# Rongjiehuang/FastDiff

Measured on AMD Instinct MI355X. Metric: real-time factor (audio-sec/wall-sec), N=4 reverse steps, 80x864 mel, higher is better.
Workload: dtype f32 results; 2-piece fp16 operands (22 bit) on fp16 MFMA, fp32 accumulate; GEMM as Winograd F(2,3); exact-fp32 twin; 1 GPU; BASELINE configs[1]: LJSpeech shape, batch=8 x 80x864 mel per GPU, N=4, HIP kernels + hipGraph sampler; batch_per_gpu=8, frames=864, reverse_steps=4, graph=True, weights=random init seed 1234 (no checkpoint offline), world_size=1, gpus_visible=1, oversubscribed=False

## Files before the change

fastdiff_amd/_capi.py:

```python
import ctypes as ct
import os

_HERE = os.path.dirname(os.path.abspath(__file__))
LIB_PATH = os.path.join(_HERE, "lib", "libfastdiff_hip.so")

FD_OK, FD_ERR_INVALID, FD_ERR_UNSUPPORTED, FD_ERR_HIP, FD_ERR_STATE, FD_ERR_MISSING = 0, -1, -2, -3, -4, -5


class FdConfig(ct.Structure):
    _fields_ = [("audio_channels", ct.c_int), ("inner_channels", ct.c_int), ("cond_channels", ct.c_int),
                ("n_upsample", ct.c_int), ("upsample_ratios", ct.c_int * 8), ("lvc_layers_each_block", ct.c_int),
                ("lvc_kernel_size", ct.c_int), ("kpnet_hidden_channels", ct.c_int), ("kpnet_conv_size", ct.c_int),
                ("diffusion_step_embed_dim_in", ct.c_int), ("diffusion_step_embed_dim_mid", ct.c_int),
                ("diffusion_step_embed_dim_out", ct.c_int), ("use_weight_norm", ct.c_int)]


class FdStep(ct.Structure):
    _fields_ = [("t", ct.c_float), ("c_eps", ct.c_float), ("c_div", ct.c_float), ("sigma", ct.c_float),
                ("c1", ct.c_float), ("c2", ct.c_float), ("c3", ct.c_float), ("add_noise", ct.c_int32)]


class FdWeightRef(ct.Structure):
    _fields_ = [("name", ct.c_char_p), ("data", ct.c_void_p), ("dims", ct.POINTER(ct.c_int64)), ("ndim", ct.c_int32), ("reserved", ct.c_int32)]


class FdKernelStat(ct.Structure):
    _fields_ = [("name", ct.c_char * 48), ("launches", ct.c_int64), ("total_ms", ct.c_double)]


class FdEmaItem(ct.Structure):
    _fields_ = [("p", ct.c_void_p), ("e", ct.c_void_p), ("numel", ct.c_int64)]


class FdEmaHyper(ct.Structure):
    _fields_ = [("decay", ct.c_double), ("warmup", ct.c_double)]


class FdEmaState(ct.Structure):
    _fields_ = [("updates", ct.c_uint64), ("seen_applied", ct.c_uint64), ("w", ct.c_float), ("apply", ct.c_int32)]


def step_table(rows):
    steps = (FdStep * len(rows))()
    for k, row in enumerate(rows):
        steps[k] = FdStep(float(row["t"]), float(row["c_eps"]), float(row["c_div"]), float(row["sigma"]),
                          float(row["c1"]), float(row["c2"]), float(row["c3"]), int(row["add_noise"]))
    return steps


EXPORTS = ["fd_default_config", "fd_create", "fd_destroy", "fd_last_error", "fd_set_weight", "fd_commit_weights",
           "fd_forward", "fd_sample", "fd_sample_check", "fd_sample_ticket", "fd_sample_settle", "fd_set_noise_streams", "fd_sample_halo_frames", "fd_sample_span", "fd_peak_normalize_int16", "fd_peak_normalize_int16_ragged", "fd_mel_spectrogram", "fd_set_mel_filterbank", "fd_get_mel_filterbank", "fd_lvc_forward", "fd_lvc_backward", "fd_lvc_forward_strided", "fd_lvc_backward_strided", "fd_gate_forward", "fd_gate_backward", "fd_kconv_forward", "fd_kconv_backward", "fd_weight_norm_multi_forward", "fd_weight_norm_multi_backward", "fd_refresh_weights_device", "fd_get_weight_image", "fd_get_weight_flags", "fd_pack_source", "fd_fan_forward", "fd_fan_backward", "fd_input_conv_forward", "fd_input_conv_backward", "fd_kconv_backward_w_multi", "fd_kconv_forward_act_multi", "fd_kconv_backward_x_multi", "fd_input_conv_forward_multi", "fd_input_conv_backward_multi", "fd_kconv_forward_act", "fd_kconv_backward_act", "fd_kconv_forward_frames", "fd_kconv_backward_frames", "fd_lvc_forward_frames", "fd_lvc_backward_frames", "fd_conv32_forward", "fd_conv32_backward", "fd_weight_norm_forward", "fd_weight_norm_backward", "fd_conv7_forward", "fd_conv7_backward", "fd_upsample_forward", "fd_upsample_backward", "fd_train_draw", "fd_train_collate", "fd_eval_collate", "fd_item_distance", "fd_eval_accumulate", "fd_mse_forward", "fd_mse_backward", "fd_adamw_multi", "fd_ema_multi", "fd_set_option", "fd_read_tap", "fd_kernel_index", "fd_bias_index",
           "fd_get_profile", "fd_reset_profile", "fd_get_counter", "fd_version", "fd_abi_revision"]

_lib = None


class FastDiffHipError(RuntimeError):
    pass


def load():
    global _lib
    if _lib is not None:
        return _lib
    if not os.path.exists(LIB_PATH):
        raise FastDiffHipError(
            f"{LIB_PATH} is missing: build it with `python -m fastdiff_amd.build` (hipcc, gfx950). "
            "fastdiff_amd has no CPU fallback.")
    lib = ct.CDLL(LIB_PATH)
    vp, ci, cf = ct.c_void_p, ct.c_int, ct.c_float
    lib.fd_version.restype = ct.c_char_p
    lib.fd_last_error.restype = ct.c_char_p
    lib.fd_last_error.argtypes = [vp]
    lib.fd_default_config.argtypes = [ct.POINTER(FdConfig)]
    lib.fd_create.argtypes = [ct.POINTER(FdConfig), ci, ct.POINTER(vp)]
    lib.fd_destroy.argtypes = [vp]
    lib.fd_set_weight.argtypes = [vp, ct.c_char_p, vp, ct.POINTER(ct.c_int64), ci]
    lib.fd_commit_weights.argtypes = [vp]
    lib.fd_refresh_weights_device.argtypes = [vp, ct.POINTER(FdWeightRef), ci, vp]
    lib.fd_get_weight_image.argtypes = [vp, vp, ct.POINTER(ct.c_size_t)]
    lib.fd_get_weight_flags.argtypes = [vp, ct.POINTER(ct.c_uint)]
    lib.fd_pack_source.argtypes = [ct.c_char_p, ci, ci, ci]
    lib.fd_forward.argtypes = [vp, vp, vp, vp, ci, ci, vp, vp, vp]
    lib.fd_sample.argtypes = [vp, vp, ci, ci, vp, ct.POINTER(FdStep), ci, ci, vp, vp, ct.c_uint64, vp, vp, vp]
# ... 27 lines not shown
    lib.fd_kconv_forward_act_multi.argtypes = [vp, ci, vp, vp, vp, ci, ci, ci, ct.c_float, vp, vp]
    lib.fd_kconv_backward_x_multi.argtypes = [vp, ci, vp, vp, vp, vp, ci, ci, ci, ct.c_float, ct.c_float, vp, vp]
    lib.fd_input_conv_forward_multi.argtypes = [vp, ci, vp, vp, vp, ci, ci, ct.c_float, vp, vp]
    lib.fd_input_conv_backward_multi.argtypes = [vp, ci, vp, vp, vp, vp, ci, ci, ct.c_float, vp, vp, vp, vp]
    lib.fd_kconv_backward_w_multi.argtypes = [vp, ci, vp, vp, vp, ci, ci, ci, ct.c_float, vp, vp, vp]
    lib.fd_kconv_forward_frames.argtypes = [vp, vp, vp, vp, ci, ci, ci, vp, vp]
    lib.fd_kconv_backward_frames.argtypes = [vp, vp, vp, vp, ci, ci, ci, vp, vp, vp, vp]
    lib.fd_lvc_forward_frames.argtypes = [vp, vp, vp, ct.c_int64, vp, ct.c_int64, ci, ci, ci, vp, vp]
    lib.fd_lvc_backward_frames.argtypes = [vp, vp, vp, ct.c_int64, vp, ci, ci, ci, vp, vp, ct.c_int64, vp, ct.c_int64, vp]
    lib.fd_conv32_forward.argtypes = [vp, vp, vp, vp, vp, ci, ct.c_int64, ci, cf, cf, vp, vp, vp]
    lib.fd_conv32_backward.argtypes = [vp, vp, vp, vp, vp, vp, ci, ct.c_int64, ci, cf, cf, vp, vp, vp, vp]
    lib.fd_conv7_forward.argtypes = [vp, ci, vp, vp, vp, ci, ct.c_int64, vp, vp]
    lib.fd_conv7_backward.argtypes = [vp, ci, vp, vp, vp, ci, ct.c_int64, vp, vp, vp, vp]
    lib.fd_upsample_forward.argtypes = [vp, vp, vp, vp, ci, ct.c_int64, ci, vp, vp]
    lib.fd_upsample_backward.argtypes = [vp, vp, vp, vp, ci, ct.c_int64, ci, vp, vp, vp, vp]
    lib.fd_weight_norm_forward.argtypes = [vp, vp, vp, ct.c_int64, ci, vp, vp, vp]
    lib.fd_weight_norm_backward.argtypes = [vp, vp, vp, vp, vp, ct.c_int64, ci, vp, vp, vp]
    lib.fd_gate_forward.argtypes = [vp, vp, vp, ci, ci, ct.c_int64, vp, vp]
    lib.fd_gate_backward.argtypes = [vp, vp, vp, ci, ci, ct.c_int64, vp, vp]
    lib.fd_train_draw.argtypes = [vp, vp, vp, ci, ci, ct.c_int64, ct.c_uint64, vp, ct.c_uint64, vp, vp, vp, vp]
    lib.fd_train_collate.argtypes = [vp, vp, vp, vp, ct.c_int64, ci, ci, ci, ct.c_uint64, vp, ct.c_uint64, ci, ci, vp, vp, vp, vp]
    lib.fd_eval_collate.argtypes = [vp, vp, vp, vp, ct.c_int64, ci, ci, ci, ct.c_uint64, vp, ct.c_uint64, vp, vp, vp, vp]
    lib.fd_item_distance.argtypes = [vp, vp, vp, ci, ct.c_int64, ci, vp, vp]
    lib.fd_eval_accumulate.argtypes = [vp, vp, vp, vp, ci, ci, ci, vp, vp, vp, vp]
    lib.fd_mse_forward.argtypes = [vp, vp, vp, ct.c_int64, vp, vp, vp]
    lib.fd_mse_backward.argtypes = [vp, vp, vp, vp, ct.c_int64, vp, vp]
    lib.fd_adamw_multi.argtypes = [vp, vp, ci, vp, vp, vp]
    lib.fd_ema_multi.argtypes = [vp, vp, ci, vp, vp, vp, vp]
    lib.fd_set_option.argtypes = [vp, ct.c_char_p, ct.c_char_p]
    lib.fd_read_tap.argtypes = [vp, ct.c_char_p, vp, ct.c_int64]
    lib.fd_read_tap.restype = ct.c_int64
    lib.fd_kernel_index.argtypes = [ci, ci, ci, ci]
    lib.fd_bias_index.argtypes = [ci, ci]
    lib.fd_get_profile.argtypes = [vp, ct.POINTER(FdKernelStat), ci]
    lib.fd_reset_profile.argtypes = [vp]
    lib.fd_get_counter.argtypes = [vp, ct.c_char_p]
    lib.fd_get_counter.restype = ct.c_int64
    _lib = lib
    return lib


def check(lib, handle, rc, what):
    if rc >= 0:
        return rc
    msg = lib.fd_last_error(handle)
    msg = msg.decode() if msg else what
    if rc == FD_ERR_INVALID:
        raise AssertionError(msg)
    if rc == FD_ERR_UNSUPPORTED:
        raise NotImplementedError(msg)
    if rc == FD_ERR_MISSING:
        raise KeyError(msg)
    raise FastDiffHipError(f"{what}: {msg} (status {rc})")
```

fastdiff_amd/csrc/fd_api_ext.cpp:

```cpp
#include <math.h>
#include <stddef.h>
#include <stdlib.h>
#include <string.h>

#include <algorithm>

#include "fd_kernels.h"
#include "fd_host.h"

extern "C" {

static const int MEL_NM = 80, MEL_NB = 513;
static std::vector<float> default_mel_bank(int variant)
{
    const double sr = 22050.0;
    const double f_sp = 200.0 / 3, min_log_hz = 1000.0, min_log_mel = min_log_hz / f_sp, logstep = log(6.4) / 27.0;
    auto hz_to_mel = [&](double f) { return f >= min_log_hz ? min_log_mel + log(f / min_log_hz) / logstep : f / f_sp; };
    auto mel_to_hz = [&](double m) { return m >= min_log_mel ? min_log_hz * exp(logstep * (m - min_log_mel)) : f_sp * m; };
    const double band[MEL_VARIANTS][2] = {{80.0, 7600.0}, {0.0, 8000.0}};
    std::vector<double> mf(MEL_NM + 2);
    const double m0 = hz_to_mel(band[variant][0]), m1 = hz_to_mel(band[variant][1]);
    for (int i = 0; i < MEL_NM + 2; ++i) mf[i] = mel_to_hz(m0 + (m1 - m0) * i / (MEL_NM + 1));
    std::vector<float> fb((size_t)MEL_NM * MEL_NB, 0.0f);
    for (int m = 0; m < MEL_NM; ++m) {
// ... 175 lines not shown
        n = (int64_t)B * T * fd::KREC; src = w.kpack + (k[5] - '0') * n;
    } else if (k.size() == 5 && k.compare(0, 4, "kp_h") == 0 && k[4] >= '0' && k[4] <= '2') {
        n = (int64_t)B * fd::HID * T; src = w.kp_hB + (k[4] - '0') * n;
    } else if (k.size() == 2 && k[0] == 'x' && k[1] >= '0' && k[1] <= '2') {
        if (!h->mode.keep_taps) FD_FAIL(h, FD_ERR_STATE, "fd_read_tap: set option taps=1 before the forward to keep block outputs");
        const int blk = k[1] - '0';
        src = w.xtap[blk]; n = (int64_t)B * fd::C * T * fd::hop(blk);
    } else if (k == "range_flags") {
        src = reinterpret_cast<const float *>(w.range_flag); n = 32;
    } else if (k == "range_flags_call") {
        src = reinterpret_cast<const float *>(w.range_flag + 64); n = 32;
    } else FD_FAIL(h, FD_ERR_INVALID, "fd_read_tap: unknown tap '%s'", name);
    if (!host_dst) return n;
    if (capacity < n) FD_FAIL(h, FD_ERR_INVALID, "fd_read_tap: capacity %lld < %lld", (long long)capacity, (long long)n);
    FD_HIP(h, hipSetDevice(h->device));
    FD_HIP(h, hipDeviceSynchronize());
    FD_HIP(h, hipMemcpy(host_dst, src, sizeof(float) * n, hipMemcpyDeviceToHost));
    return n;
}

int fd_kernel_index(int layer, int in_ch, int out_ch, int tap)
{
    if (layer < 0 || layer >= fd::LAYERS || in_ch < 0 || in_ch >= fd::C || out_ch < 0 || out_ch >= 2 * fd::C || tap < 0 || tap >= 3)
        return FD_ERR_INVALID;
    return fd::kernel_index(layer, in_ch, out_ch, tap);
}

int fd_bias_index(int layer, int out_ch)
{
    if (layer < 0 || layer >= fd::LAYERS || out_ch < 0 || out_ch >= 2 * fd::C) return FD_ERR_INVALID;
    return fd::bias_index(layer, out_ch);
}

int64_t fd_get_counter(fd_handle h, const char *name)
{
    if (!h || !name) return FD_ERR_INVALID;
    const std::string k(name);
    if (k == "pieces_redone" || k == "fp32_mask") {
        const int rcs = fd_settle(h);
        if (rcs != FD_OK) return rcs;
    }
    if (k == "pieces") return h->n_pieces;
    if (k == "pieces_redone") return h->n_pieces_redone;
    if (k == "pieces_fp32") return h->n_pieces_fp32;
    if (k == "fp32_mask") return (int64_t)h->call_fp32_mask;
    if (k == "calls_redone") return h->n_calls_redone;
    if (k == "graph_captures") return h->n_graph_captures;
    if (k == "graph_hits") return h->n_graph_hits;
    if (k == "graph_evictions") return h->n_graph_evictions;
    if (k == "weight_refreshes") return h->n_refreshes;
    if (k == "refresh_graph_drops") return h->n_refresh_graph_drops;
    if (k == "graphs_resident") return (int64_t)h->graphs.size();
    if (k == "graphs_retired") return (int64_t)h->retired.size();
    if (k == "workspace_bytes") return (int64_t)(h->ws.bytes + h->span_scratch.bytes);
    FD_FAIL(h, FD_ERR_INVALID, "fd_get_counter: unknown counter '%s'", name);
}

int fd_get_profile(fd_handle h, fd_kernel_stat *stats, int capacity)
{
    if (!h) return FD_ERR_INVALID;
    hipSetDevice(h->device);
    fd_prof_drain(h);
    int i = 0;
    for (const auto &kv : h->prof_acc) {
        if (stats && i < capacity) {
            memset(&stats[i], 0, sizeof(fd_kernel_stat));
            strncpy(stats[i].name, kv.first.c_str(), sizeof(stats[i].name) - 1);
            stats[i].launches = kv.second.first;
            stats[i].total_ms = kv.second.second;
        }
        ++i;
    }
    return i;
}

int fd_reset_profile(fd_handle h)
{
    if (!h) return FD_ERR_INVALID;
    fd_prof_drain(h);
    h->prof_acc.clear();
    return FD_OK;
}

}
```

fastdiff_amd/csrc/fd_internal.h:

```cpp
#pragma once
#include <hip/hip_runtime.h>
#include <hip/hip_ext.h>
#include <stdint.h>
#include <string.h>
#include <map>
#include <string>
#include <vector>

#include "../../include/fastdiff_hip.h"
#include "../../include/fastdiff_hip_ext.h"
#include "../../include/fastdiff_hip_train.h"

namespace fd {
constexpr int C = 32;
constexpr int COND = 80;
constexpr int HID = 64;
constexpr int NBLK = 3;
constexpr int LAYERS = 4;
constexpr int HOPT = 256;
constexpr int E_IN = 128, E_MID = 512, E_OUT = 512;
constexpr int KLAYER = 2 * C * C * 3;
constexpr int KW = KLAYER * LAYERS;
constexpr int KB = 2 * C * LAYERS;
constexpr int KREC = KW + KB;
// ... 208 lines not shown
    bool defer_check = false;
    static constexpr int STAGE_SLOTS = 8;
    struct StageSlot { char *host = nullptr; size_t cap = 0; hipEvent_t done = nullptr; };
    StageSlot stage[STAGE_SLOTS];
    unsigned stage_next = 0;
    struct SampleArgs {
        const float *mel = nullptr;
        int B = 0, T = 0, N = 0, ddim = 0;
        bool has_lens = false;
        std::vector<int> lens;
        std::vector<fd_step> table;
        const float *x_T = nullptr, *z = nullptr;
        unsigned long long seed = 0;
        float *out = nullptr, *seq_out = nullptr;
        hipStream_t stream = nullptr;
        std::vector<unsigned long long> ids;
        std::vector<long long> offs;
    };
    struct PendingCall {
        bool active = false;
        bool lazy = false;
        int slot = 0;
        long long ticket = 0;
        int B = 0, T = 0, N = 0, first = 0, count = 0;
        int T_io = 0;
        float *out = nullptr;
        hipStream_t stream = nullptr;
        StepMode mode;
        SampleArgs args;
    } pending;
    long long ticket_counter = 0;
    long long n_pieces = 0, n_pieces_redone = 0, n_pieces_fp32 = 0, n_calls_redone = 0;
    unsigned call_fp32_mask = 0;
    long long redone_ring[16] = {};
    unsigned redone_next = 0;
    int *flags_host = nullptr;
    hipEvent_t flags_done = nullptr, flags_done2 = nullptr;
    void *scratch = nullptr;
    Scratch lvc_scratch;
    Scratch kconv_scratch;
    Scratch cconv_scratch;
    Scratch span_scratch;
    Scratch step_scratch;
    std::vector<ProfEntry> prof_pending;
    std::vector<hipEvent_t> event_pool;
    std::map<std::string, std::pair<int64_t, double>> prof_acc;
};

enum Pipe { PIPE_F16_THEN_F32, PIPE_F16_ONLY, PIPE_F32_ONLY };
inline Pipe fd_pipe(const StepMode &m, bool f16_possible, int flag_word)
{
    if (!f16_possible || ((m.fp32_mask >> flag_word) & 1u)) return PIPE_F32_ONLY;
    return m.inline_fallback ? PIPE_F16_THEN_F32 : PIPE_F16_ONLY;
}
inline bool front_writes_h_image(const StepMode &m, const DevWeights &w)
{
    return m.fast[ST_KP_FRONT] && fd_pipe(m, m.conv_f16 && w.kpf_f16_ok, 19) != PIPE_F32_ONLY &&
           fd_pipe(m, m.gemm_f16 && w.gemm_f16_ok, 0) != PIPE_F32_ONLY && !(m.gemm_wino && w.gemm_w_ok);
}
inline bool last_lvc_fuses_final(const StepMode &m, const DevWeights &w)
{
    return m.fast[ST_LVC] && m.fast[ST_FINAL] && !m.keep_taps && m.fuse_final &&
           fd_pipe(m, m.lvc_f16 && w.lvc_f16_ok, 1 + 2 * fd::LAYERS + 3) != PIPE_F32_ONLY;
}

struct StepIO {
// ... 60 lines not shown
```

fastdiff_amd/csrc/fd_kernels.h:

```cpp
#pragma once
#include "fd_internal.h"

namespace fdk_fast {
constexpr int GX_CT = 4;
constexpr int GX_ROWB = 2 * 128;
constexpr int GW_PAIRS = 32;
constexpr int GW_ROWB = 1024;
__host__ __device__ inline int gx_rows(int T) { return ((T + GX_CT * 32 - 1) / (GX_CT * 32)) * (GX_CT * 32) + 2; }
__host__ __device__ inline int gw_pairs(int T) { return ((T + 2 * GW_PAIRS - 1) / (2 * GW_PAIRS)) * GW_PAIRS; }
}

namespace fdk {
hipError_t naive_first_conv(const Launch &L, const StepIO &io, int B, int T);
hipError_t naive_dblock(const Launch &L, int d, int B, int T);
hipError_t naive_kp_front(const Launch &L, const StepIO &io, int B, int T);
hipError_t naive_kp_gemm(const Launch &L, int B, int T);
hipError_t naive_convt(const Launch &L, int n, const float *x_in, float *x_out, int B, int Lin);
hipError_t naive_lvc_layer(const Launch &L, int n, int layer, float *x, const float *skip, float *y, int B, int T);
hipError_t naive_final_eps(const Launch &L, const float *x32, float *eps, int B, int T);
hipError_t naive_update(const Launch &L, float *x, const float *eps, int64_t n);
hipError_t fast_first_conv(const Launch &L, const StepIO &io, int B, int T);
hipError_t fast_dblock(const Launch &L, int d, int B, int T, const float *audio);
hipError_t fast_kp_front(const Launch &L, const StepIO &io, int B, int T);
hipError_t fast_kp_gemm(const Launch &L, int B, int T);
hipError_t fast_convt(const Launch &L, int n, const float *x_in, float *x_out, int B, int Lin);
hipError_t fast_lvc_layer(const Launch &L, const StepIO &io, int n, int layer, const float *x_in, const float *skip, float *x_out, int B, int T,
                          bool up = false);
hipError_t fast_final(const Launch &L, const StepIO &io, const float *x32, int B, int T);
bool lvc_op_needs_scratch(int Cin, int Cout, int ks, int hop);
hipError_t lvc_op_forward(const Launch &L, const float *x, const float *K, const float *bias, float *out, int B, int Cin, int Cout, int ks,
                          int T, int hop, float *scratch, int64_t kbs = 0, bool frames = false, int64_t bbs = 0);
hipError_t lvc_op_backward(const Launch &L, const float *x, const float *K, const float *dout, float *dx, float *dK, float *dbias, int B,
                           int Cin, int Cout, int ks, int T, int hop, float *scratch, int64_t kbs = 0, int64_t dkbs = 0, bool frames = false,
                           int64_t dbbs = 0);
hipError_t gate_forward(const Launch &L, const float *x, const float *y, float *out, int B, int C, int64_t len);
hipError_t gate_backward(const Launch &L, const float *y, const float *dout, float *dy, int B, int C, int64_t len);
hipError_t fan_pick(const Launch &L, const float *x, float *out, int rows, int64_t len, int f);
hipError_t fan_sum(const Launch &L, const float *const g[4], const float *gp, float *dx, int rows, int64_t len, int f);
bool kconv_supported(int M, int T);
size_t kconv_scratch_floats(int B, int M, int T);
bool kconv_frames_supported(int M, int T);
bool kconv_act_supported(int M, int T);
// ... 89 lines not shown
```

fastdiff_amd/csrc/fd_kernels_kp.hip:

```cpp
#include "fd_kernels_common.h"

namespace fdk_fast {

constexpr int KPF_VALID = 48, KPF_LDI = 68, KPF_LDH = 66;

struct KpFrontW {
    const float *in_pack[fd::NBLK], *in_b[fd::NBLK];
    const float *res_pack[fd::NBLK][6], *res_b[fd::NBLK][6];
};

__global__ void __launch_bounds__(256, 2) k_kp_front(const float *__restrict__ mel, float *__restrict__ hout, KpFrontW w,
                                                     const float *__restrict__ noise, const StepParams *params, int sampler,
                                                     int B, int T, const int *__restrict__ run_if, const int *__restrict__ lens)
{
    __shared__ float xin[fd::COND * KPF_LDI];
    if (run_if && *run_if == 0) return;
    __shared__ float h0[fd::HID * KPF_LDH];
    __shared__ float hA[fd::HID * KPF_LDH];
    __shared__ float hB[fd::HID * KPF_LDH];
    const int blk = blockIdx.z, b = blockIdx.y, t0 = blockIdx.x * KPF_VALID;
    const int Tb = frames_of(lens, b, T);
    if (t0 >= Tb) return;
    const int tid = threadIdx.x, lane = tid & 63, wave = tid >> 6, l31 = lane & 31, hi = lane >> 5;
    const int mt = wave & 1, nt = wave >> 1;
// ... 597 lines not shown
                const float bv = gb[ptile * 32 + l31] * GX_SCALE;
#pragma unroll
                for (int r = 0; r < 16; ++r) bias_lo[r] = bv;
                have_blk = cur.blk; have_xg = cur.xg;
                __builtin_amdgcn_s_waitcnt(0x0F70);
            }
            const bool more = (i + half + 1 < n_mine);
            GX_WALK_NEXT(walk, cur, more, nxt, run, left);
            const int Tb = frames_of(lens, cur.b, T);
            const bool full = (Tb % 32 == 0) || (cur.chunk * (GX_CT * 32) + GX_CT * 32 <= Tb);
            if (half == 0) {
                if (full) gx_item<0, true>(lds, cur, more, nxt, hx, kpack, wq, bias_lo, aoff, B, T, R, wave_u, lane, Tb GX_TIMING_PASS);
                else gx_item<0, false>(lds, cur, more, nxt, hx, kpack, wq, bias_lo, aoff, B, T, R, wave_u, lane, Tb GX_TIMING_PASS);
            } else {
                if (full) gx_item<1, true>(lds, cur, more, nxt, hx, kpack, wq, bias_lo, aoff, B, T, R, wave_u, lane, Tb GX_TIMING_PASS);
                else gx_item<1, false>(lds, cur, more, nxt, hx, kpack, wq, bias_lo, aoff, B, T, R, wave_u, lane, Tb GX_TIMING_PASS);
            }
            cur = nxt;
        }
    }
#ifdef FD_GX_TIMING
    ph[6] = __builtin_amdgcn_s_memtime() - t_start;
    ph[7] = __builtin_amdgcn_s_memrealtime() - r_start;
    if (lane == 0)
        for (int k = 0; k < 8; ++k) atomicAdd((unsigned long long *)&fd_gxdbg[k], (unsigned long long)ph[k]);
#endif
}

constexpr int GW_WINB = GW_PAIRS * GW_ROWB;

__global__ void __launch_bounds__(256) k_h_wino(const float *__restrict__ h, char *__restrict__ wx, int *__restrict__ range_flag, int B, int T,
                                                int P, const int *__restrict__ lens)
{
    const int bb = blockIdx.y;
    const int e = blockIdx.x * 256 + threadIdx.x, p = e >> 3, g = e & 7;
    if (p >= P) return;
    if (range_flag[32] != 0) {
        if (e == 0 && bb == 0) atomicOr(range_flag, 1);
        return;
    }
    const int Tb = frames_of(lens, bb % B, T);
    const float *hb = h + ((int64_t)bb * fd::HID + 8 * g) * T;
    const int t1 = 2 * p;
    float d[8][4];
#pragma unroll
    for (int c = 0; c < 8; ++c) {
        const float *hc = hb + (int64_t)c * T;
        d[c][0] = (t1 - 1 >= 0 && t1 - 1 < Tb) ? hc[t1 - 1] : 0.0f;
        d[c][1] = (t1 < Tb) ? hc[t1] : 0.0f;
        d[c][2] = (t1 + 1 < Tb) ? hc[t1 + 1] : 0.0f;
        d[c][3] = (t1 + 2 < Tb) ? hc[t1 + 2] : 0.0f;
    }
    float mx = 0.0f;
    char *row = wx + ((int64_t)bb * P + p) * GW_ROWB;
    const int sw = p & 15;
#pragma unroll
    for (int j = 0; j < 4; ++j) {
        float u[8];
#pragma unroll
        for (int c = 0; c < 8; ++c) {
            u[c] = j == 0 ? d[c][0] - d[c][2] : (j == 1 ? d[c][1] + d[c][2] : (j == 2 ? d[c][2] - d[c][1] : d[c][1] - d[c][3]));
            mx = fmaxf(mx, fabsf(u[c]));
        }
        float4 ph, pl;
        split8(u, ph, pl);
        *reinterpret_cast<float4 *>(row + j * 256 + ((g ^ sw) << 4)) = ph;
        *reinterpret_cast<float4 *>(row + j * 256 + (((g + 8) ^ sw) << 4)) = pl;
    }
    if (!(mx < GX_LIMIT)) atomicOr(range_flag, 1);
}

__device__ __forceinline__ void gw_dma(const char *wx, char *lds_buf, const GxItem &it, int B, int P, int wave_u, int lane)
{
#ifndef FD_GW_NO_FETCH
    gx_window_dma<GW_WINB / 4096, false>(wx + (((int64_t)it.blk * B + it.b) * P + it.chunk * GW_PAIRS) * GW_ROWB + wave_u * 1024, lds_buf, wave_u, lane);
#endif
}

template <int BUF, bool FULL>
__device__ __forceinline__ void gw_item(char *lds, const GxItem &cur, bool more, const GxItem &nxt, const char *wx, float *kpack,
                                        const float4 (&wq)[2][16], float bias_lo, const int (&aoff)[2][4], int B, int T, int P,
                                        int wave_u, int lane, int Tb)
{
    const int l31 = lane & 31, hi = lane >> 5;
    if (more) gw_dma(wx, lds + (BUF ^ 1) * GW_WINB, nxt, B, P, wave_u, lane);
    const int t_begin = cur.chunk * (2 * GW_PAIRS);
    float *krow = kpack + (((int64_t)cur.blk * B + cur.b) * T + t_begin) * fd::KREC + (cur.xg * 4 + wave_u) * 32;
    const unsigned loff = (unsigned)(8 * hi) * (unsigned)fd::KREC + (unsigned)l31;
    const __amdgpu_buffer_rsrc_t rs = __builtin_amdgcn_make_buffer_rsrc(krow, 0, 2 * GW_PAIRS * fd::KREC * 4, 0x00020000);
    const f32x16 zero = {0.f, 0.f, 0.f, 0.f, 0.f, 0.f, 0.f, 0.f, 0.f, 0.f, 0.f, 0.f, 0.f, 0.f, 0.f, 0.f};
    const char *hb = lds + BUF * GW_WINB;
    constexpr int ORDER[4] = {1, 2, 0, 3};
    f32x16 keep, acc, lo;
#pragma unroll
    for (int r = 0; r < 16; ++r) lo[r] = bias_lo;
    float4 a1, a2;
    auto store16 = [&](int odd) {
#ifdef FD_GX_NO_STORE
        if (FULL) {
#pragma unroll
            for (int r = 0; r < 16; ++r) { const float v_ = fmaf(lo[r], GX_INV_SCALE, acc[r]); asm volatile("" :: "v"(v_)); }
            (void)rs; (void)loff;
            return;
        }
#endif
        if (FULL) {
#pragma unroll
            for (int r = 0; r < 16; ++r) {
                acc[r] = fmaf(lo[r], GX_INV_SCALE, acc[r]);
                __builtin_amdgcn_raw_buffer_store_b32(__float_as_uint(acc[r]), rs, loff * 4u, (2 * ((r & 3) + 8 * (r >> 2)) + odd) * fd::KREC * 4,
                                                      FD_GX_STORE_AUX);
            }
        } else {
#pragma unroll
            for (int r = 0; r < 16; ++r)
                if (t_begin + 2 * drow(r, hi) + odd < Tb) (krow + (2 * ((r & 3) + 8 * (r >> 2)) + odd) * fd::KREC)[loff] = fmaf(lo[r], GX_INV_SCALE, acc[r]);
        }
    };
#pragma unroll
    for (int s = 0; s < 4; ++s) {
        const int j = ORDER[s];
        a1 = *reinterpret_cast<const float4 *>(hb + aoff[0][0] + j * 256);
        a2 = *reinterpret_cast<const float4 *>(hb + aoff[1][0] + j * 256);
#pragma unroll
        for (int k4 = 0; k4 < 4; ++k4) {
            const int kg = j * 4 + k4;
            float4 n1 = a1, n2 = a2;
            if (k4 + 1 < 4) {
                n1 = *reinterpret_cast<const float4 *>(hb + aoff[0][k4 + 1] + j * 256);
                n2 = *reinterpret_cast<const float4 *>(hb + aoff[1][k4 + 1] + j * 256);
            }
            acc = mfma_f16(a1, wq[0][kg], (k4 == 0 && s == 0) ? zero : ((k4 == 0 && s == 3) ? keep : acc));
            lo = mfma_f16(a2, wq[0][kg], (k4 == 0 && s == 3) ? zero : lo);
            lo = mfma_f16(a1, wq[1][kg], lo);
            a1 = n1;
            a2 = n2;
        }
        if (s == 0) {
#pragma unroll
            for (int r = 0; r < 16; ++r) keep[r] = fmaf(lo[r], GX_INV_SCALE, acc[r]);
        } else if (s == 1) {
#pragma unroll
            for (int r = 0; r < 16; ++r) keep[r] = fmaf(2.0f, keep[r], -fmaf(lo[r], GX_INV_SCALE, acc[r]));
        } else store16(s == 3 ? 1 : 0);
    }
    if (more) {
#ifdef FD_GX_NO_STORE
        asm volatile("s_waitcnt vmcnt(0)" ::: "memory");
#else
        if (FULL) asm volatile("s_waitcnt vmcnt(32)" ::: "memory");
        else asm volatile("s_waitcnt vmcnt(0)" ::: "memory");
#endif
    }
    __builtin_amdgcn_s_barrier();
}

__global__ void __launch_bounds__(256, 2) k_kp_gemm_w(const char *__restrict__ wx , float *__restrict__ kpack,
                                                      const float4 *g0, const float4 *g1, const float4 *g2, const float *gb0,
                                                      const float *gb1, const float *gb2, const int *__restrict__ range_flag, int B,
                                                      int T, int P, int chunks_per_utt, int n_items, const int *__restrict__ lens)
{
    __shared__ __attribute__((aligned(16))) char lds[2 * GW_WINB];
    const int tid = threadIdx.x, lane = tid & 63, l31 = lane & 31, hi = lane >> 5;
    const int wave_u = __builtin_amdgcn_readfirstlane(tid >> 6);
    if (*range_flag != 0) return;
    GxWalk walk(B, chunks_per_utt, n_items, gridDim.x, blockIdx.x);
    const int n_mine = walk.n_mine;
    if (n_mine <= 0) return;
    int run = 0, left = walk.left0;
    GxItem cur = walk.first();
    int aoff[2][4];
#pragma unroll
    for (int q2 = 0; q2 < 2; ++q2)
#pragma unroll
        for (int k4 = 0; k4 < 4; ++k4) aoff[q2][k4] = l31 * GW_ROWB + (((q2 * 8 + k4 * 2 + hi) ^ (l31 & 15)) << 4);
    gw_dma(wx, lds, cur, B, P, wave_u, lane);
    asm volatile("s_waitcnt vmcnt(0)" ::: "memory");
    __builtin_amdgcn_s_barrier();
    float4 wq[2][16];
    float bias_lo = 0.0f;
    int have_blk = -1, have_xg = -1;
#pragma unroll 1
    for (int i = 0; i < n_mine; i += 2) {
#pragma unroll
        for (int half = 0; half < 2; ++half) {
            if (half == 1 && i + 1 >= n_mine) break;
            if (cur.blk != have_blk || cur.xg != have_xg) {
                const float4 *gp = cur.blk == 0 ? g0 : (cur.blk == 1 ? g1 : g2);
                const float *gb = cur.blk == 0 ? gb0 : (cur.blk == 1 ? gb1 : gb2);
                const int ptile = cur.xg * 4 + wave_u;
#pragma unroll
                for (int q2 = 0; q2 < 2; ++q2)
#pragma unroll
                    for (int kg = 0; kg < 16; ++kg) wq[q2][kg] = gp[(((int64_t)ptile * 2 + q2) * 16 + kg) * 64 + lane];
                bias_lo = gb[ptile * 32 + l31] * GX_SCALE;
                have_blk = cur.blk; have_xg = cur.xg;
                __builtin_amdgcn_s_waitcnt(0x0F70);
            }
            const bool more = (i + half + 1 < n_mine);
            GX_WALK_NEXT(walk, cur, more, nxt, run, left);
            const int Tb = frames_of(lens, cur.b, T);
            const bool full = cur.chunk * (2 * GW_PAIRS) + 2 * GW_PAIRS <= Tb;
            if (half == 0) {
                if (full) gw_item<0, true>(lds, cur, more, nxt, wx, kpack, wq, bias_lo, aoff, B, T, P, wave_u, lane, Tb);
                else gw_item<0, false>(lds, cur, more, nxt, wx, kpack, wq, bias_lo, aoff, B, T, P, wave_u, lane, Tb);
            } else {
                if (full) gw_item<1, true>(lds, cur, more, nxt, wx, kpack, wq, bias_lo, aoff, B, T, P, wave_u, lane, Tb);
                else gw_item<1, false>(lds, cur, more, nxt, wx, kpack, wq, bias_lo, aoff, B, T, P, wave_u, lane, Tb);
            }
            cur = nxt;
        }
    }
}

}

namespace fdk {
using namespace fdk_fast;

hipError_t fast_kp_front(const Launch &L, const StepIO &io, int B, int T)
{
    fd_context *c = L.ctx;
    const DevWeights &w = c->w;
    const dim3 grid((T + KPF_VALID - 1) / KPF_VALID, B, fd::NBLK);
    const StepMode &m = *L.mode;
    const int *lens = m.ragged ? c->ws.lens_dev : nullptr;
    const int *run_if = nullptr;
    const char *name = "kp_front";
    const Pipe pipe = fd_pipe(m, m.conv_f16 && w.kpf_f16_ok, 19);
    if (pipe != PIPE_F32_ONLY) {
        KpFrontW2 k2;
        for (int n = 0; n < fd::NBLK; ++n) {
            k2.in_pack[n] = reinterpret_cast<const float4 *>(w.kp_in_h2[n]); k2.in_b[n] = w.blk[n].kp_in.b;
            for (int l = 0; l < 6; ++l) { k2.res_pack[n][l] = reinterpret_cast<const float4 *>(w.kp_res_h2[n][l]); k2.res_b[n][l] = w.blk[n].kp_res[l].b; }
        }
        const bool image = front_writes_h_image(m, w);
        FD_LAUNCH(L, name, k_kp_front_h2, grid, dim3(256), 0, io.mel, c->ws.kp_hB, image ? reinterpret_cast<char *>(c->ws.h_f16) : (char *)nullptr, k2,
                  (const float *)c->ws.noise, (const StepParams *)c->ws.params, io.sampler, B, T, gx_rows(T), c->ws.range_flag, lens);
        run_if = c->ws.range_flag + 19;
        name = "kp_front_fp32_fallback";
        if (pipe == PIPE_F16_ONLY) return hipSuccess;
    }
    KpFrontW kw;
    for (int n = 0; n < fd::NBLK; ++n) {
        kw.in_pack[n] = w.kp_in_pack[n]; kw.in_b[n] = w.blk[n].kp_in.b;
        for (int l = 0; l < 6; ++l) { kw.res_pack[n][l] = w.kp_res_pack[n][l]; kw.res_b[n][l] = w.blk[n].kp_res[l].b; }
    }
    FD_LAUNCH(L, name, k_kp_front, grid, dim3(256), 0, io.mel, c->ws.kp_hB, kw, (const float *)c->ws.noise,
              (const StepParams *)c->ws.params, io.sampler, B, T, run_if, lens);
    return hipSuccess;
}

struct GemmGrid { int chunks, items, grid; };
static GemmGrid gemm_grid(const fd_context *c, int B, int chunks)
{
    const int items = fd::NBLK * (fd::KREC / 128) * B * chunks;
    return {chunks, items, items < 2 * c->num_cus ? items : 2 * c->num_cus};
}

hipError_t fast_kp_gemm(const Launch &L, int B, int T)
{
    fd_context *c = L.ctx;
    const DevWeights &w = c->w;
    const StepMode &m = *L.mode;
    const int *lens = m.ragged ? c->ws.lens_dev : nullptr;
    const Pipe pipe = fd_pipe(m, m.gemm_f16 && w.gemm_f16_ok, 0);
    const bool f16 = pipe != PIPE_F32_ONLY;
    if (f16 && m.gemm_wino && w.gemm_w_ok) {
        const int P = gw_pairs(T);
        const GemmGrid g = gemm_grid(c, B, P / GW_PAIRS);
        FD_LAUNCH(L, "h_wino", k_h_wino, dim3((8 * P + 255) / 256, fd::NBLK * B), dim3(256), 0, (const float *)c->ws.kp_hB,
                  reinterpret_cast<char *>(c->ws.h_f16), c->ws.range_flag, B, T, P, lens);
        FD_LAUNCH(L, "kp_gemm_f16x2", k_kp_gemm_w, dim3(g.grid), dim3(256), 0, reinterpret_cast<const char *>(c->ws.h_f16), c->ws.kpack,
                  reinterpret_cast<const float4 *>(w.gemm_w_pack[0]), reinterpret_cast<const float4 *>(w.gemm_w_pack[1]),
                  reinterpret_cast<const float4 *>(w.gemm_w_pack[2]), w.gemm_bias[0], w.gemm_bias[1], w.gemm_bias[2],
                  (const int *)c->ws.range_flag, B, T, P, g.chunks, g.items, lens);
        if (pipe == PIPE_F16_ONLY) return hipSuccess;
    } else if (f16) {
        const int R = gx_rows(T);
        const GemmGrid g = gemm_grid(c, B, (T + GX_CT * 32 - 1) / (GX_CT * 32));
        if (!front_writes_h_image(m, w))
            FD_LAUNCH(L, "h_split", k_h_split, dim3((32 * R + 255) / 256, fd::NBLK * B), dim3(256), 0, (const float *)c->ws.kp_hB,
                      reinterpret_cast<unsigned *>(c->ws.h_f16), c->ws.range_flag, B, T, R, lens);
        FD_LAUNCH(L, "kp_gemm_f16x2", k_kp_gemm_h2, dim3(g.grid), dim3(256), 0, reinterpret_cast<const char *>(c->ws.h_f16), c->ws.kpack,
                  reinterpret_cast<const float4 *>(w.gemm_h2_pack[0]), reinterpret_cast<const float4 *>(w.gemm_h2_pack[1]),
                  reinterpret_cast<const float4 *>(w.gemm_h2_pack[2]), w.gemm_bias[0], w.gemm_bias[1], w.gemm_bias[2],
                  (const int *)c->ws.range_flag, B, T, R, g.chunks, g.items, lens);
        if (pipe == PIPE_F16_ONLY) return hipSuccess;
    }
    const int tiles_per_utt = (T + 31) / 32;
    const GemmGrid g = gemm_grid(c, B, (tiles_per_utt + GEMM_CT - 1) / GEMM_CT);
    const int chunk_tiles = (tiles_per_utt + g.chunks - 1) / g.chunks;
    FD_LAUNCH(L, f16 ? "kp_gemm_fp32_fallback" : "kp_gemm", k_kp_gemm, dim3(g.grid), dim3(256), 0, (const float *)c->ws.kp_hB, c->ws.kpack,
              w.gemm_pack[0], w.gemm_pack[1], w.gemm_pack[2], w.gemm_bias[0], w.gemm_bias[1], w.gemm_bias[2], B, T, g.chunks,
              chunk_tiles, g.items, f16 ? (const int *)c->ws.range_flag : (const int *)nullptr, lens);
    return hipSuccess;
}

}
```

include/fastdiff_hip_ext.h:

```cpp
#ifndef FASTDIFF_HIP_EXT_H
#define FASTDIFF_HIP_EXT_H

#include "fastdiff_hip.h"

#ifdef __cplusplus
extern "C" {
#endif

FD_API int fd_peak_normalize_int16(fd_handle h, const float *wav, int B, int64_t L, int16_t *pcm, void *stream);
FD_API int fd_peak_normalize_int16_ragged(fd_handle h, const float *wav, int B, int64_t L, const int64_t *valid, int16_t *pcm,
                                          void *stream);

FD_API int fd_mel_spectrogram(fd_handle h, const float *wav, int B, int64_t n_samples, float *mel, int T, void *stream);

FD_API int fd_set_mel_filterbank(fd_handle h, const float *fb, int n_mels, int n_bins);
FD_API int fd_get_mel_filterbank(fd_handle h, float *fb_out, int n_mels, int n_bins);


FD_API int fd_sample_halo_frames(int N);

FD_API int fd_sample_span(fd_handle h, const float *mel, int64_t mel_first, int64_t mel_frames, int64_t utt_frames, int64_t t0, int64_t t1,
                          const fd_step *table, int N, int ddim, const float *x_T, const float *z, uint64_t seed, uint64_t stream_id,
                          int window_frames, float *out, void *stream);

typedef struct fd_weight_ref {
    const char *name;
    const float *data;
    const int64_t *dims;
    int32_t ndim, reserved;
} fd_weight_ref;
FD_API int fd_refresh_weights_device(fd_handle h, const fd_weight_ref *items, int n, void *stream);


FD_API int fd_get_weight_image(fd_handle h, void *host_buf, size_t *nbytes);
FD_API int fd_get_weight_flags(fd_handle h, unsigned *ok_mask);
FD_API int fd_pack_source(const char *pack, int p0, int p1, int pos);

FD_API int64_t fd_read_tap(fd_handle h, const char *name, float *host_dst, int64_t capacity);

FD_API int fd_kernel_index(int layer, int in_ch, int out_ch, int tap);
FD_API int fd_bias_index(int layer, int out_ch);

typedef struct fd_kernel_stat {
    char name[48];
    int64_t launches;
    double total_ms;
} fd_kernel_stat;
FD_API int fd_get_profile(fd_handle h, fd_kernel_stat *stats, int capacity);
FD_API int fd_reset_profile(fd_handle h);

FD_API int64_t fd_get_counter(fd_handle h, const char *name);

#ifdef __cplusplus
}
#endif
#endif
```

Baseline: 9839 x real-time.

## Flatten Winograd kernel-predictor GEMM across batch to remove per-utterance padding

When every utterance has the same length (no lens array), the Winograd h transform and the f16x2 kernel-predictor GEMM now treat the whole batch as one flat sequence of output pairs instead of padding each utterance to a multiple of GW_PAIRS. This cuts the padded tail tiles per utterance and gives more uniform work items. Partial tiles now carry row-mapping metadata (cut, phase, reciprocal) and use masked buffer stores. The non-full path now waits on vmcnt(32) instead of 0. It also adds a geometry query and counters for testing.

Measured after the change: 9902 x real-time (median of 6 runs). Within noise of the previous version (+0.6%).

```diff
diff --git a/fastdiff_amd/_capi.py b/fastdiff_amd/_capi.py
--- a/fastdiff_amd/_capi.py
+++ b/fastdiff_amd/_capi.py
@@ -49,7 +49,7 @@
 
 
 EXPORTS = ["fd_default_config", "fd_create", "fd_destroy", "fd_last_error", "fd_set_weight", "fd_commit_weights",
-           "fd_forward", "fd_sample", "fd_sample_check", "fd_sample_ticket", "fd_sample_settle", "fd_set_noise_streams", "fd_sample_halo_frames", "fd_sample_span", "fd_peak_normalize_int16", "fd_peak_normalize_int16_ragged", "fd_mel_spectrogram", "fd_set_mel_filterbank", "fd_get_mel_filterbank", "fd_lvc_forward", "fd_lvc_backward", "fd_lvc_forward_strided", "fd_lvc_backward_strided", "fd_gate_forward", "fd_gate_backward", "fd_kconv_forward", "fd_kconv_backward", "fd_weight_norm_multi_forward", "fd_weight_norm_multi_backward", "fd_refresh_weights_device", "fd_get_weight_image", "fd_get_weight_flags", "fd_pack_source", "fd_fan_forward", "fd_fan_backward", "fd_input_conv_forward", "fd_input_conv_backward", "fd_kconv_backward_w_multi", "fd_kconv_forward_act_multi", "fd_kconv_backward_x_multi", "fd_input_conv_forward_multi", "fd_input_conv_backward_multi", "fd_kconv_forward_act", "fd_kconv_backward_act", "fd_kconv_forward_frames", "fd_kconv_backward_frames", "fd_lvc_forward_frames", "fd_lvc_backward_frames", "fd_conv32_forward", "fd_conv32_backward", "fd_weight_norm_forward", "fd_weight_norm_backward", "fd_conv7_forward", "fd_conv7_backward", "fd_upsample_forward", "fd_upsample_backward", "fd_train_draw", "fd_train_collate", "fd_eval_collate", "fd_item_distance", "fd_eval_accumulate", "fd_mse_forward", "fd_mse_backward", "fd_adamw_multi", "fd_ema_multi", "fd_set_option", "fd_read_tap", "fd_kernel_index", "fd_bias_index",
+           "fd_forward", "fd_sample", "fd_sample_check", "fd_sample_ticket", "fd_sample_settle", "fd_set_noise_streams", "fd_sample_halo_frames", "fd_sample_span", "fd_peak_normalize_int16", "fd_peak_normalize_int16_ragged", "fd_mel_spectrogram", "fd_set_mel_filterbank", "fd_get_mel_filterbank", "fd_lvc_forward", "fd_lvc_backward", "fd_lvc_forward_strided", "fd_lvc_backward_strided", "fd_gate_forward", "fd_gate_backward", "fd_kconv_forward", "fd_kconv_backward", "fd_weight_norm_multi_forward", "fd_weight_norm_multi_backward", "fd_refresh_weights_device", "fd_get_weight_image", "fd_get_weight_flags", "fd_pack_source", "fd_fan_forward", "fd_fan_backward", "fd_input_conv_forward", "fd_input_conv_backward", "fd_kconv_backward_w_multi", "fd_kconv_forward_act_multi", "fd_kconv_backward_x_multi", "fd_input_conv_forward_multi", "fd_input_conv_backward_multi", "fd_kconv_forward_act", "fd_kconv_backward_act", "fd_kconv_forward_frames", "fd_kconv_backward_frames", "fd_lvc_forward_frames", "fd_lvc_backward_frames", "fd_conv32_forward", "fd_conv32_backward", "fd_weight_norm_forward", "fd_weight_norm_backward", "fd_conv7_forward", "fd_conv7_backward", "fd_upsample_forward", "fd_upsample_backward", "fd_train_draw", "fd_train_collate", "fd_eval_collate", "fd_item_distance", "fd_eval_accumulate", "fd_mse_forward", "fd_mse_backward", "fd_adamw_multi", "fd_ema_multi", "fd_set_option", "fd_read_tap", "fd_kernel_index", "fd_bias_index", "fd_gemm_geometry",
            "fd_get_profile", "fd_reset_profile", "fd_get_counter", "fd_version", "fd_abi_revision"]
 
 _lib = None
@@ -143,6 +143,7 @@
     lib.fd_read_tap.restype = ct.c_int64
     lib.fd_kernel_index.argtypes = [ci, ci, ci, ci]
     lib.fd_bias_index.argtypes = [ci, ci]
+    lib.fd_gemm_geometry.argtypes = [ci, ci, ci, ci, ct.POINTER(ci)]
     lib.fd_get_profile.argtypes = [vp, ct.POINTER(FdKernelStat), ci]
     lib.fd_reset_profile.argtypes = [vp]
     lib.fd_get_counter.argtypes = [vp, ct.c_char_p]
diff --git a/fastdiff_amd/csrc/fd_api_ext.cpp b/fastdiff_amd/csrc/fd_api_ext.cpp
--- a/fastdiff_amd/csrc/fd_api_ext.cpp
+++ b/fastdiff_amd/csrc/fd_api_ext.cpp
@@ -231,6 +231,21 @@
     return fd::bias_index(layer, out_ch);
 }
 
+int fd_gemm_geometry(int B, int T, int ragged, int q, int *out)
+{
+    using namespace fdk_fast;
+    if (B < 1 || T < 1 || !out || (int64_t)B * T >= (1 << 24)) return FD_ERR_INVALID;
+    const int entries = ragged ? B : 1, P = ragged ? gw_pairs(T) : gw_pairs_flat(B, T);
+    out[0] = P;
+    out[1] = entries * (P / GW_PAIRS);
+    out[2] = out[3] = -1;
+    if (ragged || q < 0 || q >= B * gw_half(T)) return FD_OK;
+    const int row = gw_record_row(q, T), b = q / gw_half(T);
+    out[2] = row;
+    out[3] = (row + 1 < (b + 1) * T) ? row + 1 : -1;
+    return FD_OK;
+}
+
 int64_t fd_get_counter(fd_handle h, const char *name)
 {
     if (!h || !name) return FD_ERR_INVALID;
@@ -251,6 +266,8 @@
     if (k == "refresh_graph_drops") return h->n_refresh_graph_drops;
     if (k == "graphs_resident") return (int64_t)h->graphs.size();
     if (k == "graphs_retired") return (int64_t)h->retired.size();
+    if (k == "gemm_items") return h->gemm_items;
+    if (k == "gemm_flat") return h->gemm_flat ? 1 : 0;
     if (k == "workspace_bytes") return (int64_t)(h->ws.bytes + h->span_scratch.bytes);
     FD_FAIL(h, FD_ERR_INVALID, "fd_get_counter: unknown counter '%s'", name);
 }
diff --git a/fastdiff_amd/csrc/fd_internal.h b/fastdiff_amd/csrc/fd_internal.h
--- a/fastdiff_amd/csrc/fd_internal.h
+++ b/fastdiff_amd/csrc/fd_internal.h
@@ -264,6 +264,8 @@
     long long ticket_counter = 0;
     long long n_pieces = 0, n_pieces_redone = 0, n_pieces_fp32 = 0, n_calls_redone = 0;
     unsigned call_fp32_mask = 0;
+    int gemm_items = 0;
+    bool gemm_flat = false;
     long long redone_ring[16] = {};
     unsigned redone_next = 0;
     int *flags_host = nullptr;
diff --git a/fastdiff_amd/csrc/fd_kernels.h b/fastdiff_amd/csrc/fd_kernels.h
--- a/fastdiff_amd/csrc/fd_kernels.h
+++ b/fastdiff_amd/csrc/fd_kernels.h
@@ -8,6 +8,9 @@
 constexpr int GW_ROWB = 1024;
 __host__ __device__ inline int gx_rows(int T) { return ((T + GX_CT * 32 - 1) / (GX_CT * 32)) * (GX_CT * 32) + 2; }
 __host__ __device__ inline int gw_pairs(int T) { return ((T + 2 * GW_PAIRS - 1) / (2 * GW_PAIRS)) * GW_PAIRS; }
+__host__ __device__ inline int gw_half(int T) { return (T + 1) / 2; }
+__host__ __device__ inline int gw_pairs_flat(int B, int T) { return ((B * gw_half(T) + GW_PAIRS - 1) / GW_PAIRS) * GW_PAIRS; }
+__host__ __device__ inline int gw_record_row(int q, int T) { const int b = q / gw_half(T); return b * T + 2 * (q - b * gw_half(T)); }
 }
 
 namespace fdk {
diff --git a/fastdiff_amd/csrc/fd_kernels_kp.hip b/fastdiff_amd/csrc/fd_kernels_kp.hip
--- a/fastdiff_amd/csrc/fd_kernels_kp.hip
+++ b/fastdiff_amd/csrc/fd_kernels_kp.hip
@@ -653,14 +653,20 @@
 __global__ void __launch_bounds__(256) k_h_wino(const float *__restrict__ h, char *__restrict__ wx, int *__restrict__ range_flag, int B, int T,
                                                 int P, const int *__restrict__ lens)
 {
-    const int bb = blockIdx.y;
-    const int e = blockIdx.x * 256 + threadIdx.x, p = e >> 3, g = e & 7;
-    if (p >= P) return;
+    const int e = blockIdx.x * 256 + threadIdx.x, q = e >> 3, g = e & 7;
+    if (q >= P) return;
     if (range_flag[32] != 0) {
-        if (e == 0 && bb == 0) atomicOr(range_flag, 1);
+        if (e == 0 && blockIdx.y == 0) atomicOr(range_flag, 1);
         return;
     }
-    const int Tb = frames_of(lens, bb % B, T);
+    int bb = blockIdx.y, p = q, Tb;
+    if (lens) Tb = lens[bb % B];
+    else {
+        const int b = q / gw_half(T);
+        p = q - b * gw_half(T);
+        Tb = b < B ? T : 0;
+        bb = blockIdx.y * B + (b < B ? b : 0);
+    }
     const float *hb = h + ((int64_t)bb * fd::HID + 8 * g) * T;
     const int t1 = 2 * p;
     float d[8][4];
@@ -673,8 +679,8 @@
         d[c][3] = (t1 + 2 < Tb) ? hc[t1 + 2] : 0.0f;
     }
     float mx = 0.0f;
-    char *row = wx + ((int64_t)bb * P + p) * GW_ROWB;
-    const int sw = p & 15;
+    char *row = wx + ((int64_t)blockIdx.y * P + q) * GW_ROWB;
+    const int sw = q & 15;
 #pragma unroll
     for (int j = 0; j < 4; ++j) {
         float u[8];
@@ -698,15 +704,15 @@
 #endif
 }
 
+struct GwRows { int row0, lim, cut, ph, rcp; };
 template <int BUF, bool FULL>
 __device__ __forceinline__ void gw_item(char *lds, const GxItem &cur, bool more, const GxItem &nxt, const char *wx, float *kpack,
                                         const float4 (&wq)[2][16], float bias_lo, const int (&aoff)[2][4], int B, int T, int P,
-                                        int wave_u, int lane, int Tb)
+                                        int wave_u, int lane, const GwRows &rows)
 {
     const int l31 = lane & 31, hi = lane >> 5;
     if (more) gw_dma(wx, lds + (BUF ^ 1) * GW_WINB, nxt, B, P, wave_u, lane);
-    const int t_begin = cur.chunk * (2 * GW_PAIRS);
-    float *krow = kpack + (((int64_t)cur.blk * B + cur.b) * T + t_begin) * fd::KREC + (cur.xg * 4 + wave_u) * 32;
+    float *krow = kpack + (((int64_t)cur.blk * B + cur.b) * T + rows.row0) * fd::KREC + (cur.xg * 4 + wave_u) * 32;
     const unsigned loff = (unsigned)(8 * hi) * (unsigned)fd::KREC + (unsigned)l31;
     const __amdgpu_buffer_rsrc_t rs = __builtin_amdgcn_make_buffer_rsrc(krow, 0, 2 * GW_PAIRS * fd::KREC * 4, 0x00020000);
     const f32x16 zero = {0.f, 0.f, 0.f, 0.f, 0.f, 0.f, 0.f, 0.f, 0.f, 0.f, 0.f, 0.f, 0.f, 0.f, 0.f, 0.f};
@@ -734,8 +740,20 @@
             }
         } else {
 #pragma unroll
-            for (int r = 0; r < 16; ++r)
-                if (t_begin + 2 * drow(r, hi) + odd < Tb) (krow + (2 * ((r & 3) + 8 * (r >> 2)) + odd) * fd::KREC)[loff] = fmaf(lo[r], GX_INV_SCALE, acc[r]);
+            for (int r = 0; r < 16; ++r) {
+                const int d = drow(r, hi);
+                int sub = d >= rows.cut, last = d == rows.cut - 1;
+                if (rows.ph) {
+                    const int pp = d + rows.ph - rows.cut;
+                    sub = (pp * rows.rcp) >> 16;
+                    last = pp - sub * rows.ph == rows.ph - 1;
+                }
+                const int rel = 2 * d - sub + odd;
+                const bool live = rel < rows.lim && !(odd && last);
+                acc[r] = fmaf(lo[r], GX_INV_SCALE, acc[r]);
+                __builtin_amdgcn_raw_buffer_store_b32(__float_as_uint(acc[r]), rs, live ? ((unsigned)rel * (unsigned)fd::KREC + (unsigned)l31) * 4u : 0x80000000u,
+                                                      0, FD_GX_STORE_AUX);
+            }
         }
     };
 #pragma unroll
@@ -769,8 +787,7 @@
 #ifdef FD_GX_NO_STORE
         asm volatile("s_waitcnt vmcnt(0)" ::: "memory");
 #else
-        if (FULL) asm volatile("s_waitcnt vmcnt(32)" ::: "memory");
-        else asm volatile("s_waitcnt vmcnt(0)" ::: "memory");
+        asm volatile("s_waitcnt vmcnt(32)" ::: "memory");
 #endif
     }
     __builtin_amdgcn_s_barrier();
@@ -779,7 +796,8 @@
 __global__ void __launch_bounds__(256, 2) k_kp_gemm_w(const char *__restrict__ wx , float *__restrict__ kpack,
                                                       const float4 *g0, const float4 *g1, const float4 *g2, const float *gb0,
                                                       const float *gb1, const float *gb2, const int *__restrict__ range_flag, int B,
-                                                      int T, int P, int chunks_per_utt, int n_items, const int *__restrict__ lens)
+                                                      int T, int P, int chunks_per_utt, int n_items, const int *__restrict__ lens,
+                                                      int flat_T)
 {
     __shared__ __attribute__((aligned(16))) char lds[2 * GW_WINB];
     const int tid = threadIdx.x, lane = tid & 63, l31 = lane & 31, hi = lane >> 5;
@@ -821,13 +839,23 @@
             const bool more = (i + half + 1 < n_mine);
             GX_WALK_NEXT(walk, cur, more, nxt, run, left);
             const int Tb = frames_of(lens, cur.b, T);
-            const bool full = cur.chunk * (2 * GW_PAIRS) + 2 * GW_PAIRS <= Tb;
+            GwRows rows = {cur.chunk * (2 * GW_PAIRS), 0, 1 << 30, 0, 0};
+            bool full = rows.row0 + 2 * GW_PAIRS <= Tb;
+            if (flat_T) {
+                const int half = gw_half(flat_T), q0 = cur.chunk * GW_PAIRS, p0 = q0 % half;
+                rows.row0 = gw_record_row(q0, flat_T);
+                rows.cut = half - p0;
+                rows.ph = half < GW_PAIRS ? half : 0;
+                rows.rcp = (65536 + half - 1) / half;
+                full = rows.cut > GW_PAIRS;
+            }
+            rows.lim = Tb - rows.row0;
             if (half == 0) {
-                if (full) gw_item<0, true>(lds, cur, more, nxt, wx, kpack, wq, bias_lo, aoff, B, T, P, wave_u, lane, Tb);
-                else gw_item<0, false>(lds, cur, more, nxt, wx, kpack, wq, bias_lo, aoff, B, T, P, wave_u, lane, Tb);
+                if (full) gw_item<0, true>(lds, cur, more, nxt, wx, kpack, wq, bias_lo, aoff, B, T, P, wave_u, lane, rows);
+                else gw_item<0, false>(lds, cur, more, nxt, wx, kpack, wq, bias_lo, aoff, B, T, P, wave_u, lane, rows);
             } else {
-                if (full) gw_item<1, true>(lds, cur, more, nxt, wx, kpack, wq, bias_lo, aoff, B, T, P, wave_u, lane, Tb);
-                else gw_item<1, false>(lds, cur, more, nxt, wx, kpack, wq, bias_lo, aoff, B, T, P, wave_u, lane, Tb);
+                if (full) gw_item<1, true>(lds, cur, more, nxt, wx, kpack, wq, bias_lo, aoff, B, T, P, wave_u, lane, rows);
+                else gw_item<1, false>(lds, cur, more, nxt, wx, kpack, wq, bias_lo, aoff, B, T, P, wave_u, lane, rows);
             }
             cur = nxt;
         }
@@ -888,14 +916,18 @@
     const Pipe pipe = fd_pipe(m, m.gemm_f16 && w.gemm_f16_ok, 0);
     const bool f16 = pipe != PIPE_F32_ONLY;
     if (f16 && m.gemm_wino && w.gemm_w_ok) {
-        const int P = gw_pairs(T);
-        const GemmGrid g = gemm_grid(c, B, P / GW_PAIRS);
-        FD_LAUNCH(L, "h_wino", k_h_wino, dim3((8 * P + 255) / 256, fd::NBLK * B), dim3(256), 0, (const float *)c->ws.kp_hB,
+        const bool flat = lens == nullptr;
+        const int P = flat ? gw_pairs_flat(B, T) : gw_pairs(T);
+        const int entries = flat ? 1 : B, frames = flat ? B * T : T;
+        const GemmGrid g = gemm_grid(c, entries, P / GW_PAIRS);
+        FD_LAUNCH(L, "h_wino", k_h_wino, dim3((8 * P + 255) / 256, fd::NBLK * entries), dim3(256), 0, (const float *)c->ws.kp_hB,
                   reinterpret_cast<char *>(c->ws.h_f16), c->ws.range_flag, B, T, P, lens);
         FD_LAUNCH(L, "kp_gemm_f16x2", k_kp_gemm_w, dim3(g.grid), dim3(256), 0, reinterpret_cast<const char *>(c->ws.h_f16), c->ws.kpack,
                   reinterpret_cast<const float4 *>(w.gemm_w_pack[0]), reinterpret_cast<const float4 *>(w.gemm_w_pack[1]),
                   reinterpret_cast<const float4 *>(w.gemm_w_pack[2]), w.gemm_bias[0], w.gemm_bias[1], w.gemm_bias[2],
-                  (const int *)c->ws.range_flag, B, T, P, g.chunks, g.items, lens);
+                  (const int *)c->ws.range_flag, entries, frames, P, g.chunks, g.items, lens, flat && (T & 1) ? T : 0);
+        c->gemm_items = entries * g.chunks;
+        c->gemm_flat = flat;
         if (pipe == PIPE_F16_ONLY) return hipSuccess;
     } else if (f16) {
         const int R = gx_rows(T);
diff --git a/include/fastdiff_hip_ext.h b/include/fastdiff_hip_ext.h
--- a/include/fastdiff_hip_ext.h
+++ b/include/fastdiff_hip_ext.h
@@ -41,6 +41,8 @@
 FD_API int fd_kernel_index(int layer, int in_ch, int out_ch, int tap);
 FD_API int fd_bias_index(int layer, int out_ch);
 
+FD_API int fd_gemm_geometry(int B, int T, int ragged, int q, int *out);
+
 typedef struct fd_kernel_stat {
     char name[48];
     int64_t launches;
```
